# auduno/headtrackr

Measured on AMD Instinct MI355X. Metric: frames/sec full-cascade detect at 320x240, higher is better.
Workload: dtype u8; 1 GPU; C2: 256 x 320x240 RGBA frames per GPU, full BBF cascade detect (interval 5) incl. grouping + best face per frame on the host; frames_per_gpu=256, frames_total=256, width=320, height=240, batches_in_flight=3, parallelism=1 GPU

## Files before the change

### headtrackr_amd/csrc/ht_context.hip

```cpp
#include <sched.h>
#include <algorithm>
#include <cmath>
#include <cstddef>
#include <cstdlib>
#include <cstring>
#include <new>

#include "ht_internal.h"
#include "ht_hostpost.h"
#include "ht_geometry_plan.h"
#include "ht_cascade_plan.h"

static thread_local std::string g_create_err;

#include <dlfcn.h>
namespace {
struct Roctx {
    int (*push)(const char *) = nullptr;
    int (*pop)() = nullptr;
    Roctx() {
        void *h = dlopen("libroctx64.so", RTLD_NOW | RTLD_GLOBAL);
        if (!h) h = dlopen("libroctx64.so.4", RTLD_NOW | RTLD_GLOBAL);
        if (h) {
            push = reinterpret_cast<int (*)(const char *)>(dlsym(h, "roctxRangePushA"));
// ... 105 lines not shown
    ctx->timers[idx].launches++;
}

extern "C" int32_t ht_abi_version(void) { return HT_ABI_VERSION; }

extern "C" const char *ht_last_error(const ht_ctx *ctx) { return ctx ? ctx->err.c_str() : g_create_err.c_str(); }

static bool apply_options(ht_ctx *c, const std::string &opts, std::string &why) {
    size_t pos = 0;
    while (pos < opts.size()) {
        size_t end = opts.find(',', pos);
        if (end == std::string::npos) end = opts.size();
        std::string kv = opts.substr(pos, end - pos);
        pos = end + 1;
        while (!kv.empty() && (kv.front() == ' ')) kv.erase(kv.begin());
        while (!kv.empty() && (kv.back() == ' ')) kv.pop_back();
        if (kv.empty()) continue;
        const size_t eq = kv.find('=');
        const std::string key = kv.substr(0, eq), val = eq == std::string::npos ? "1" : kv.substr(eq + 1);
        char *endp = nullptr;
        const long long v = std::strtoll(val.c_str(), &endp, 10);
        if (val.empty() || (endp && *endp)) {
            why = "option '" + key + "': value is not an integer";
            return false;
        }
        const int iv = (int)std::max<long long>(std::min<long long>(v, 1ll << 30), -(1ll << 30));
        if (key == "rs_rpt") { if (iv >= 1 && iv <= HT_RS_MAX_PASSES) c->rs_rpt = iv; }
        else if (key == "rs_tailtable") c->tail_table = iv < 0 ? 0 : (iv > 2 ? 2 : (int)iv), c->tail_table_forced = true;
        else if (key == "rs_tailcap") c->rs_tailcap = (uint64_t)std::max<long long>(v, 0), c->rs_tailcap_forced = true;
        else if (key == "rs_notail") c->rs_notail = iv != 0;
        else if (key == "rs_nofast") c->rs_nofast = iv != 0;
        else if (key == "rs_nosort") c->rs_nosort = iv != 0;
        else if (key == "rs_bands") c->rs_bands = iv != 0;
        else if (key == "rs_gennames") c->rs_gennames = iv != 0;
        else if (key == "rs_minwg") c->rs_min_wgs = std::max(1, iv);
        else if (key == "rs_k") c->dbg_rs_k = iv;
        else if (key == "rs_group") { if (iv >= 1 && iv <= 64) c->rs_group = iv, c->rs_group_forced = true; }
        else if (key == "early_scan") c->early_scan = iv != 0;
        else if (key == "force_exact") c->dbg_force_exact = iv;
        else if (key == "deep_bias") c->deep_bias = (uint32_t)std::max(0, iv);
        else if (key == "deep_v") c->dbg_deep_v = iv;
        else if (key == "cs_flags") c->cs_flags = iv != 0;
        else if (key == "cs_sync_ring") c->cs_sync_ring = iv != 0;
        else if (key == "cs_pairs_force") c->cs_pairs_force = iv != 0;
        else if (key == "cs_pairs_cluster") c->cs_pairs_cluster = iv != 0;
        else if (key == "fp_sparse") c->fp_sparse = iv != 0;
        else if (key == "deep_grid") c->deep_grid = std::max(1, iv);
        else if (key == "split") c->opt_split = std::max(1, iv);
        else if (key == "cs_fused_min") c->cs_fused_min_streams = std::max(1, iv);
        else if (key == "cs_fused_nt") c->cs_fused_nt = iv;
        else if (key == "cs_keep_hist") c->cs_keep_hist = iv != 0;
        else if (key == "cs_seq_fused") c->cs_seq_fused = iv != 0;
        else if (key == "cs_cluster") c->cs_cluster = iv != 0;
        else if (key == "cs_cluster_min_px") c->cs_cluster_min_px = (uint32_t)std::max(0, iv);
        else if (key == "cs_region") c->cs_region_cap = std::min(40960, std::max(0, iv));
        else if (key == "cs_barrier_budget") c->cs_barrier_budget = std::max(1ll, v);
        else if (key == "graph_max_frames") c->graph_max_frames = std::max(0, iv);
        else if (key == "host_threads") c->host_threads = std::min(64, std::max(0, iv));
        else if (key == "force_rccl") c->force_rccl = iv != 0;
        else if (key == "group_cap") c->grp_cap_opt = std::max(1, iv);
#ifdef HT_DEBUG_KNOBS
        else if (key == "stop_stage") c->dbg_stop_stage = iv;
        else if (key == "cs_iters") c->dbg_cs_iters = std::min(10, std::max(0, iv));
        else if (key == "rs_maxgen") c->rs_maxgen = iv;
#endif
        else {
// ... 169 lines not shown
    ht_cs_best_free(c);
    ht_cs_faces_free(c);
    ht_group_free(c);
    if (c->d_gather) (void)hipFree(c->d_gather);
    for (auto &a : release) {
        if (a.orphan) {
            (void)hipSetDevice(a.device);
            (void)hipDeviceSynchronize();
        }
        (void)hipFree(a.p);
    }
    (void)hipSetDevice(c->device);
    for (auto &t : c->timers)
        for (auto &p : t.pending) (void)hipEventDestroy(p.first), (void)hipEventDestroy(p.second);
    if (c->own_stream && c->stream) (void)hipStreamDestroy(c->stream);
    delete c;
}


static ht_status set_geometry_impl(ht_ctx *c, int32_t width, int32_t height, int32_t max_batch, const int32_t *level_dims, int n, int upto) {
    c->W = width;
    c->H = height;
    c->max_batch = max_batch;
    c->nlevels = n;
    c->upto = upto;

    HtPlanInputs in;
    in.interval = c->interval, in.next = c->next, in.cw = c->cascade.cw, in.ch = c->cascade.ch;
    in.rs_rpt = c->rs_rpt, in.rs_nofast = c->rs_nofast, in.rs_nosort = c->rs_nosort, in.rs_notail = c->rs_notail;
    in.rs_tailcap = c->rs_tailcap, in.rs_tailcap_forced = c->rs_tailcap_forced;
    in.tail_table = c->tail_table, in.tail_table_forced = c->tail_table_forced;
    in.early_scan = c->early_scan, in.aux_stream = c->aux_stream != nullptr;
    in.queue_capacity_cfg = c->queue_capacity_cfg;
    HtGeometryPlan &P = c->plan;
    std::string why;
    ht_status st = ht_plan_geometry(in, width, height, max_batch, level_dims, n, upto, &P, &why);
    if (st != HT_OK) return ht_fail(c, st, why);

    c->d_gen_blocks.assign(P.gens.size(), nullptr);
    for (size_t g = 1; g < P.gens.size(); g++)
        if ((st = upload_table(c, c->d_gen_blocks[g], P.gen_tiles[g])) != HT_OK) return st;
    HT_HIP(c, hipMalloc(&c->d_levels, sizeof(HtDevLevel) * HT_MAX_LEVELS));
    HT_HIP(c, hipMemcpy(c->d_levels, P.levels, sizeof(HtDevLevel) * n, hipMemcpyHostToDevice));
    if (hipMalloc(&c->d_arena, P.arena_stride * (uint64_t)max_batch) != hipSuccess)
        return ht_fail(c, HT_ERR_NOMEM, "ht_set_geometry: hipMalloc(pyramid arena) failed");
    HT_HIP(c, hipMemset(c->d_arena, 0, P.arena_stride * (uint64_t)max_batch));
    if ((st = upload_table(c, c->d_tail_jobs, P.tail_jobs)) != HT_OK || (st = upload_table(c, c->d_tail_prefix, P.tail_prefix)) != HT_OK ||
        (st = upload_table(c, c->d_tail_taps, P.tail_taps)) != HT_OK || (st = upload_table(c, c->d_tail_taps_fast, P.tail_taps_fast)) != HT_OK ||
        (st = upload_table(c, c->d_tail_tapref, P.tail_tapref)) != HT_OK || (st = upload_table(c, c->d_tile_recs, P.tile_recs)) != HT_OK ||
        (st = upload_table(c, c->d_scales, P.scales)) != HT_OK)
        return st;
    if (hipMalloc(&c->d_queue, (size_t)P.queue_capacity * sizeof(HtQueueEntry) + HT_DEEP_CTR_BYTES) != hipSuccess)
        return ht_fail(c, HT_ERR_NOMEM, "ht_set_geometry: hipMalloc(survivor queue) failed");
    return HT_OK;
}

extern "C" ht_status ht_set_geometry(ht_ctx *c, int32_t width, int32_t height, int32_t max_batch, const int32_t *level_dims,
                                     int32_t nlevels_in) {
    if (!c) return HT_ERR_INVALID;
    if (width <= 0 || height <= 0 || width > 16384 || height > 16384 || max_batch <= 0)
        return ht_fail(c, HT_ERR_INVALID, "ht_set_geometry: width/height must be 1..16384 and max_batch > 0");
    HT_HIP(c, hipSetDevice(c->device));
    const int upto = (int)std::floor(std::log((double)std::min(c->cascade.cw, c->cascade.ch)) / std::log(ht_scale_of(c->interval)));
    const int n = upto + c->next * 2;
    if (n > HT_MAX_LEVELS) return ht_fail(c, HT_ERR_INVALID, "ht_set_geometry: too many pyramid levels");
    if (level_dims && nlevels_in != n) return ht_fail(c, HT_ERR_INVALID, "ht_set_geometry: level_dims has the wrong number of levels");
// ... 631 lines not shown
```

### headtrackr_amd/csrc/ht_geometry_plan.h

```cpp
#pragma once

#include <algorithm>
#include <cmath>
#include <cstring>
#include <string>
#include <vector>

#include "ht_hostpost.h"
#include "ht_plan_types.h"

static inline uint64_t align_up(uint64_t v, uint64_t a) { return (v + a - 1) / a * a; }

static HtTap ht_host_tap(int i, double r, int s, int origin) {
    double f = ((double)i + 0.5) * r;
    f = f + (-0.5);
    f = f < 0.0 ? 0.0 : f;
    const double fmax = (double)(s - 1);
    f = f > fmax ? fmax : f;
    const double af = std::floor(f);
    HtTap tp;
    tp.a = origin + (int)af;
    tp.b = origin + std::min((int)af + 1, s - 1);
    tp.t = f - af;
    tp.u = 1.0 - tp.t;
// ... 55 lines not shown
        j.dst_stride = D.stride;
        j.sx = sx, j.sy = sy, j.sw = sw, j.sh = sh;
        j.dw = dw, j.dh = dh;
        j.cw = D.w, j.ch = D.h;
        if (sw <= 0 || sh <= 0 || dw <= 0 || dh <= 0) {
            j.dw = j.dh = 0;
            j.sw = j.sh = 1;
            j.rx = j.ry = 1;
        } else {
            j.rx = (double)sw / (double)dw;
            j.ry = (double)sh / (double)dh;
        }
        p->gens[g].push_back(j);
    };
    for (int i = 1; i < n; i++) {
        const HtDevLevel &D = p->levels[i];
        if (i <= in.interval) {
            add_job(gen[i], 0, i, 0, 0, 0, p->levels[0].w, p->levels[0].h, D.w, D.h);
        } else {
            const HtDevLevel &S = p->levels[i - next];
            add_job(gen[i], i - next, i, 0, 0, 0, S.w, S.h, D.w, D.h);
            if (i >= 2 * next) {
                add_job(gen[i], i - next, i, 1, 1, 0, S.w - 1, S.h, D.w - 2, D.h);
                add_job(gen[i], i - next, i, 2, 0, 1, S.w, S.h - 1, D.w, D.h - 2);
                add_job(gen[i], i - next, i, 3, 1, 1, S.w - 1, S.h - 1, D.w - 2, D.h - 2);
            }
        }
    }
}

static std::vector<HtResampleJob> ht_plan_gen_tiles(const HtPlanInputs &in, const std::vector<HtResampleJob> &jobs) {
    std::vector<HtResampleJob> tiles;
    for (auto &j : jobs) {
        int npmax = 1;
        for (int t = 2; t <= std::min(in.rs_rpt, HT_RS_MAX_PASSES); t++)
            if ((int)std::ceil(16.0 * t * j.ry) + 3 <= HT_RS_SRC_ROWS) npmax = t;
        const int passes = (j.ch + 15) / 16, nby = (passes + npmax - 1) / npmax, nbx = (j.cw + 63) / 64;
        int pass0 = 0;
        for (int y = 0; y < nby; y++) {
            const int np = passes / nby + (y < passes % nby ? 1 : 0);
            for (int x = 0; x < nbx; x++) {
                HtResampleJob t = j;
                t.bx = (uint16_t)x, t.pass0 = (uint16_t)pass0, t.np = (uint16_t)np;
                t.pad = in.rs_nofast ? 2 : (uint16_t)((j.dw > 0 && j.sw == 2 * j.dw && j.sh == 2 * j.dh) ? 1 : 0);
                const int X0 = 64 * x, Y0 = 16 * pass0, ncols = std::min(64, j.dw - X0), nrows = std::min(16 * np, j.dh - Y0);
                if (ncols > 0 && nrows > 0) {
                    t.ex_xa = ht_host_tap(X0, j.rx, j.sw, j.sx).a & ~15;
                    t.ex_ya = ht_host_tap(Y0, j.ry, j.sh, j.sy).a;
                    t.ex_sw16 = (ht_host_tap(X0 + ncols - 1, j.rx, j.sw, j.sx).b - t.ex_xa) / 16 + 1;
                    t.ex_sh = ht_host_tap(Y0 + nrows - 1, j.ry, j.sh, j.sy).b - t.ex_ya + 1;
                    bool fit = t.ex_sw16 * 16 <= 160;
                    for (int w = 0; w < 4; w++) {
                        const int r0 = std::min(4 * np * w, nrows - 1), r1 = std::min(4 * np * (w + 1) - 1, nrows - 1);
                        const int bya = ht_host_tap(Y0 + r0, j.ry, j.sh, j.sy).a - t.ex_ya;
                        const int bsh = ht_host_tap(Y0 + r1, j.ry, j.sh, j.sy).b - (t.ex_ya + bya) + 1;
                        if (bya < 0 || bya > 255 || bsh < 1 || bsh > HT_RSB_ROWS) fit = false;
                        t.band_ya4 |= (uint32_t)(bya & 0xff) << (8 * w), t.band_sh4 |= (uint32_t)(bsh & 0xff) << (8 * w);
                    }
                    if (fit) t.pad |= 4;
                }
                tiles.push_back(t);
            }
            pass0 += np;
        }
    }
    if (!in.rs_nosort)
        std::stable_sort(tiles.begin(), tiles.end(), [](const HtResampleJob &a, const HtResampleJob &b) {
            if (a.src_off != b.src_off) return a.src_off < b.src_off;
            const int ya = (int)(16.0 * a.pass0 * a.ry), yb = (int)(16.0 * b.pass0 * b.ry);
            if (ya / 32 != yb / 32) return ya < yb;
            return a.bx < b.bx;
        });
    return tiles;
}

static void ht_plan_tail(const HtPlanInputs &in, int max_batch, HtGeometryPlan *p) {
    const int ngen = (int)p->gens.size();
    constexpr int HT_SMALL_BATCH = 48;
    const uint64_t tail_cap = in.rs_tailcap_forced ? in.rs_tailcap : (max_batch <= HT_SMALL_BATCH ? 4000u : in.rs_tailcap);
    p->tail_table = in.tail_table_forced ? in.tail_table : ((max_batch <= 128 && max_batch > HT_SMALL_BATCH) ? 1 : 0);
    p->tail_first_gen = 0;
    if (in.rs_notail) return;
    int g0 = ngen;
    uint64_t px = 0;
    for (int g = ngen - 1; g >= 1; g--) {
        uint64_t gp = 0;
        for (auto &j : p->gens[g]) gp += (uint64_t)j.cw * j.ch;
        if (p->gens[g].size() > (size_t)HT_TAIL_MAX_JOBS || px + gp > tail_cap) break;
        px += gp;
        g0 = g;
    }
    if (!(ngen - g0 >= 2 && ngen - g0 <= HT_TAIL_MAX_GENS)) return;
    std::vector<HtResampleJob> &tj = p->tail_jobs;
    std::vector<uint32_t> &pref = p->tail_prefix;
    HtTailGens &T = p->tail;
    std::memset(&T, 0, sizeof(T));
    T.ngen = ngen - g0;
    for (int g = g0; g < ngen; g++) {
        T.job_begin[g - g0] = (int32_t)tj.size();
        uint32_t groups = 0;
        for (auto &j : p->gens[g]) {
            tj.push_back(j);
            pref.push_back(groups);
            groups += (uint32_t)((j.cw + 3) / 4) * (uint32_t)j.ch;
// ... 128 lines not shown
```

### headtrackr_amd/csrc/ht_internal.h

```cpp
#pragma once

#include <hip/hip_runtime.h>
#include <stdint.h>

#include <atomic>
#include <string>
#include <vector>

#include "headtrackr_hip.h"

#include "ht_cascade_types.h"

#include "ht_plan_types.h"

constexpr int HT_TAIL_LDS_TAPS = 4096;

struct HtBlockRef {
    uint16_t item;
    uint16_t bx, by;
    uint16_t pad;
};

struct alignas(16) HtQueueEntry {
    uint32_t frame;
// ... 75 lines not shown
    bool builtin_cascade = false;
    uint32_t deep_bias = 1;
    int dbg_stop_stage = -1, dbg_force_exact = 0, dbg_deep_v = 4, deep_grid = 192;
    HtDevStage *d_stages = nullptr;
    int opt_split = 0;

    int W = 0, H = 0, max_batch = 0, nlevels = 0, upto = 0;
    HtGeometryPlan plan;
    HtDevLevel *d_levels = nullptr;
    uint8_t *d_arena = nullptr;
    std::vector<HtResampleJob *> d_gen_blocks;
    HtTileRec *d_tile_recs = nullptr;
    HtScanScale *d_scales = nullptr;
    HtResampleJob *d_tail_jobs = nullptr;
    uint32_t *d_tail_prefix = nullptr;
    HtTap *d_tail_taps = nullptr;
    HtTapFast *d_tail_taps_fast = nullptr;
    HtTailTapRef *d_tail_tapref = nullptr;
    bool deep_attr_set = false;
    int tail_table = 1;
    bool tail_table_forced = false;
    bool rs_nofast = false, rs_nosort = false, rs_notail = false, rs_gennames = false;
    uint64_t rs_tailcap = 32768;
    bool rs_tailcap_forced = false;
    int rs_maxgen = 1 << 30;
    bool force_rccl = false;
    int host_threads = -1;
    int rs_min_wgs = 1536;
    int dbg_rs_k = 0;
    int rs_group = 8;
    bool rs_group_forced = false;
    int rs_rpt = 4;
    bool rs_bands = true;

    uint8_t *d_frames_own = nullptr;
    size_t d_frames_own_bytes = 0;
    uint8_t *d_frames_back = nullptr;
    size_t d_frames_back_bytes = 0;
    int back_n = 0;
    hipStream_t copy_stream = nullptr;
    hipEvent_t ev_copy_done = nullptr, ev_front_free = nullptr;
    const uint8_t *d_frames = nullptr;
    size_t frame_stride = 0;
    int nframes = 0;
    std::atomic<bool> capturing{false};
    int graph_max_frames = 256;
    std::vector<HtDetectGraph> graphs;
    uint64_t graph_launches = 0;
    int64_t requeue_flags = -1;
    int enq_nframes = 0;

    uint32_t hit_capacity = 1u << 20, queue_capacity_cfg = 0;
    ht_hit *d_hits = nullptr;
    HtQueueEntry *d_queue = nullptr;
    HtCounters *d_counters = nullptr;
    uint32_t spec_hint = 0;
    HtCounters h_counters;
    uint8_t *h_pinned = nullptr;
    unsigned long long *d_stats = nullptr;
    unsigned long long h_stage_in[64] = {0};
    std::vector<ht_hit> h_collect_hits;
    std::vector<uint32_t> h_collect_counts;
    std::vector<ht_hit> h_raw_hits;
    std::vector<ht_hit> h_ordered_hits;
    std::vector<uint32_t> h_frame_start;
    bool stats_enqueued = false;
// ... 224 lines not shown
```

### headtrackr_amd/csrc/ht_plan_types.h

```cpp
#pragma once

#include <stdint.h>

#include <vector>

#include "headtrackr_hip.h"

struct HtDevLevel {
    int32_t w, h, stride;
    uint32_t off[4];
};

constexpr int HT_TAIL_MAX_GENS = 8;
constexpr int HT_TAIL_MAX_JOBS = 32;
struct HtTailGens {
    int32_t ngen;
    int32_t job_begin[HT_TAIL_MAX_GENS + 1];
    uint32_t groups[HT_TAIL_MAX_GENS];
    uint32_t tap_begin[HT_TAIL_MAX_GENS + 1];
};

struct HtTap {
    double t, u;
    int32_t a, b;
};
struct HtTapFast {
    int32_t a;
    float tf;
};
struct HtTailTapRef {
    uint32_t col, row;
    uint32_t mode;
    uint32_t pad;
};

constexpr int HT_RS_SRC_ROWS = 75;
constexpr int HT_RS_MAX_PASSES = 4;
struct HtResampleJob {
    uint32_t src_off, dst_off;
    int32_t src_stride, dst_stride;
    int32_t sx, sy, sw, sh;
    int32_t dw, dh;
    int32_t cw, ch;
    uint16_t bx, pass0;
    uint16_t np, pad;
    double rx, ry;
    int32_t ex_xa, ex_ya;
    int32_t ex_sw16, ex_sh;
    uint32_t band_ya4, band_sh4;
};
constexpr int HT_RSB_ROWS = 24;

constexpr int HT_SCAN_TXH = 64;
constexpr int HT_SCAN_TYH = 32;
struct HtScanScale {
    int32_t l0, l1, l2;
    int32_t qw, qh;
    int32_t tw2, th2;
    int32_t ntx, nty;
    uint32_t tile_begin;
    uint32_t div_magic;
    uint32_t win_begin;
};

struct alignas(64) HtTileRec {
    uint32_t off0, off1, off2[4];
    uint32_t sh0, sh1, sh2;
    uint32_t origin;
    uint32_t size;
    uint32_t tw2_l0;
    uint32_t div_magic;
    uint32_t strip_magic;
    uint32_t pad[2];
};
static_assert(sizeof(HtTileRec) == 64, "HtTileRec");

struct HtPlanInputs {
    int interval, next;
    uint32_t cw, ch;
    int rs_rpt;
    bool rs_nofast, rs_nosort, rs_notail;
    uint64_t rs_tailcap;
    bool rs_tailcap_forced;
    int tail_table;
    bool tail_table_forced;
    bool early_scan, aux_stream;
    uint32_t queue_capacity_cfg;
};

struct HtGeometryPlan {
    HtDevLevel levels[HT_MAX_LEVELS] = {};
    uint64_t arena_stride = 0;
    uint64_t pyr_bytes = 0, windows_per_frame = 0;
    std::vector<std::vector<HtResampleJob>> gens;
    std::vector<std::vector<HtResampleJob>> gen_tiles;
    std::vector<uint32_t> gen_blocks;
    int tail_first_gen = 0;
    int tail_table = 0;
    std::vector<HtResampleJob> tail_jobs;
    std::vector<uint32_t> tail_prefix;
    std::vector<HtTap> tail_taps;
    std::vector<HtTapFast> tail_taps_fast;
    std::vector<HtTailTapRef> tail_tapref;
    HtTailGens tail = {};
    std::vector<HtScanScale> scales;
    std::vector<HtTileRec> tile_recs;
    uint32_t tiles_per_frame = 0;
    int early_gen = 0;
    uint32_t early_tiles = 0;
    uint32_t queue_capacity = 0;
};
```

### headtrackr_amd/csrc/ht_pyramid.hip

```cpp
#include <cstdio>
#include <cstdlib>
#include <cstring>
#include <type_traits>

#include "ht_internal.h"
#include "ht_resample_tap.h"
#define HT_GRAY_FN __device__ __forceinline__
#include "ht_gray.h"

namespace {

__device__ __forceinline__ bool xcd_item(uint32_t per_frame, uint32_t nframes, uint32_t *frame, uint32_t *item) {
    const uint32_t chunk = gridDim.x >> 3;
    const uint32_t t = (blockIdx.x & 7u) * chunk + (blockIdx.x >> 3);
    if (t >= per_frame * nframes) return false;
    *frame = t / per_frame;
    *item = t - *frame * per_frame;
    return true;
}

__device__ __forceinline__ uint32_t gray_of(uint32_t px) { return ht_gray_of(px); }

template <bool GRAY_IN_R, bool WB>
__global__ __launch_bounds__(256) void k_gray_linear(const uint8_t *__restrict__ frames, size_t frame_stride,
// ... 71 lines not shown

typedef unsigned int rs_u32x4 __attribute__((ext_vector_type(4)));
typedef float rs_f2 __attribute__((ext_vector_type(2)));
__device__ __forceinline__ uint4 rs_buf_load16(__amdgpu_buffer_rsrc_t r, uint32_t voff, uint32_t soff) {
    const rs_u32x4 v = __builtin_amdgcn_raw_buffer_load_b128(r, voff, soff, 0);
    return make_uint4(v.x, v.y, v.z, v.w);
}

template <typename PTR>
__device__ __forceinline__ uint32_t rs_pixels4(PTR r0, PTR r1, const RsTap (&cx)[4], const RsTap &ry, int xoff, int npx) {
    uint32_t o = 0;
#pragma unroll
    for (int k = 0; k < 4; k++) {
        if (k < npx) {
            const int ia = cx[k].a - xoff, ib = cx[k].b - xoff;
            const double top = __dadd_rn(__dmul_rn((double)r0[ia], cx[k].u), __dmul_rn((double)r0[ib], cx[k].t));
            const double bot = __dadd_rn(__dmul_rn((double)r1[ia], cx[k].u), __dmul_rn((double)r1[ib], cx[k].t));
            const double vv = __dadd_rn(__dmul_rn(top, ry.u), __dmul_rn(bot, ry.t));
            const int q = (int)__builtin_rint(vv);
            o |= (uint32_t)q << (8 * k);
        }
    }
    return o;
}

#define RS_LDS_BARRIER()                                                     \
    do {                                                                     \
        __builtin_amdgcn_fence(__ATOMIC_RELEASE, "workgroup", "local");      \
        __builtin_amdgcn_s_barrier();                                        \
        __builtin_amdgcn_fence(__ATOMIC_ACQUIRE, "workgroup", "local");      \
    } while (0)
#define RS_LD1(ptr_) __hip_atomic_load((ptr_), __ATOMIC_RELAXED, __HIP_MEMORY_SCOPE_WORKGROUP)

__device__ __forceinline__ uint32_t rs_pixel_f64(const uint8_t *p, const uint8_t *p1, double cu, double ct, double ru, double rt) {
    const double top = __dadd_rn(__dmul_rn((double)p[0], cu), __dmul_rn((double)p1[0], ct));
    const double bot = __dadd_rn(__dmul_rn((double)p[RS_SP], cu), __dmul_rn((double)p1[RS_SP], ct));
    const double vv = __dadd_rn(__dmul_rn(top, ru), __dmul_rn(bot, rt));
    return (uint32_t)__double2loint(__dadd_rn(vv, 6755399441055744.0));
}

constexpr float RS_EPS = 1.0f / 8192.0f;

constexpr int RS_WPS = 6;
#if defined(HT_RS_PHASES)
__device__ unsigned long long g_rs_tl[16384][8][8];
__device__ unsigned long long g_rs_launch[1024][4];
__device__ unsigned long long g_rs_tw[4096][4][6];
#define RS_WSTAMP(i)                                                                                                                  \
    do {                                                                                                                              \
        __builtin_amdgcn_sched_barrier(0);                                                                                            \
        if (rs_iter == 2u && (threadIdx.x & 63u) == 0) g_rs_tw[rs_slot & 4095u][threadIdx.x >> 6][i] = __builtin_readcyclecounter(); \
        __builtin_amdgcn_sched_barrier(0);                                                                                            \
    } while (0)
#define HT_RS_TIMELINE 1
#define RS_SUB(i)                                                                       \
    do {                                                                                \
        __builtin_amdgcn_sched_barrier(0);                                              \
        if (threadIdx.x == 0) g_rs_tl[rs_slot][7][i] = __builtin_readcyclecounter();    \
        __builtin_amdgcn_sched_barrier(0);                                              \
    } while (0)
#define RS_STAMP(i)                                                                     \
    do {                                                                                \
        __builtin_amdgcn_sched_barrier(0);                                              \
        if (threadIdx.x == 0) g_rs_tl[rs_slot][rs_iter & 7u][i] = __builtin_readcyclecounter(); \
        __builtin_amdgcn_sched_barrier(0);                                              \
    } while (0)
#elif defined(HT_RS_TIMELINE)
__device__ unsigned long long g_rs_timeline[1 << 16][8];
#define RS_STAMP(i)                                                                     \
// ... 264 lines not shown
        int ytl = yt;
        asm volatile("" : "+v"(ytl));
#pragma unroll
        for (int q = 0; q < RPT; q++) {
            const int y = ytl + 16 * q;
            uint32_t o = 0;
            if (drawn && q < np && y < Jm.dh && npx > 0) {
                const RsTap ry = rs_tap(y, Jm.ry, Jm.sh, Jm.sy);
                o = rs_pixels4<const uint8_t *>(src + (size_t)ry.a * Jm.src_stride, src + (size_t)ry.b * Jm.src_stride, cx, ry, 0, npx);
            }
            if (q < np && y < Jm.ch && x0 < Jm.dst_stride) *reinterpret_cast<uint32_t *>(frame + Jm.dst_off + (size_t)y * Jm.dst_stride + x0) = o;
        }
    }
}

constexpr int RSB_WPS = 8;
constexpr int RSB_BAND = 4096;
#if defined(HT_RS_PHASES)
__device__ unsigned long long g_rsb_ph[256][8];
#define RSB_T(var_)                                     \
    do {                                                \
        __builtin_amdgcn_sched_barrier(0);              \
        var_ = __builtin_readcyclecounter();            \
        __builtin_amdgcn_sched_barrier(0);              \
    } while (0)
#else
#define RSB_T(var_)
#endif
typedef __attribute__((address_space(3))) void rs_lds_void;
template <int RPT>
__global__ __launch_bounds__(256, RSB_WPS) void k_resample_bands(const HtResampleJob *__restrict__ tiles, uint8_t *__restrict__ arena,
                                                                    uint64_t arena_stride, uint32_t blocks_per_frame, uint32_t ngroups,
                                                                    uint32_t nframes, uint32_t group_frames) {
    constexpr int TH = 16 * RPT;
    __shared__ __attribute__((aligned(16))) uint8_t s_src[4 * RSB_BAND];
    __shared__ RsTap s_col[RS_TW], s_row[TH];
    uint32_t gidx, blk;
    if (!xcd_item(blocks_per_frame, ngroups, &gidx, &blk)) return;
#ifdef HT_RS_PHASES
    unsigned long long rsb_t_entry = 0, rsb_t0 = 0, rsb_t1 = 0, rsb_t2 = 0, rsb_t3 = 0, rsb_t4 = 0, rsb_acc[7] = {0, 0, 0, 0, 0, 0, 0};
    RSB_T(rsb_t_entry);
#endif
    const HtResampleJob J = tiles[blk];
    const uint32_t f0 = gidx * group_frames, f1 = min(f0 + group_frames, nframes);
    const int tid = (int)threadIdx.x;
    const int np = (int)J.np;
    const int X0 = (int)J.bx * RS_TW, Y0 = (int)J.pass0 * 16;
    uint8_t *frame = arena + (uint64_t)f0 * arena_stride;
    const int ncols = min(RS_TW, J.dw - X0), nrows = min(16 * np, J.dh - Y0);
    const uint32_t mode = J.pad;
    if ((mode & 4u) && ncols > 0 && nrows > 0) {
        const int w = __builtin_amdgcn_readfirstlane(tid >> 6), l = tid & 63;
        const int xa = J.ex_xa, sw16 = J.ex_sw16;
        const int yaw = J.ex_ya + (int)((J.band_ya4 >> (8 * w)) & 0xffu);
        const int bsh = (int)((J.band_sh4 >> (8 * w)) & 0xffu);
        uint8_t *const band = s_src + w * RSB_BAND;
        uint32_t voff[4];
        bool on[4];
#pragma unroll
        for (int i = 0; i < 4; i++) {
            const int c = i * 64 + l, row = (c * 205) >> 11, col = c - row * 10;
            on[i] = col < sw16 && row < bsh;
            voff[i] = J.src_off + (uint32_t)((yaw + row) * J.src_stride + xa + 16 * col);
        }
        uint64_t fbase = reinterpret_cast<uint64_t>(frame);
#define RS_FRAME_RSRC(base_) __builtin_amdgcn_make_buffer_rsrc(reinterpret_cast<void *>(base_), 0, (int)0xffffffffu, 0x00020000)
#define RSB_DMA(fr_, soff_)                                                                                                              \
    do {                                                                                                                                 \
        _Pragma("unroll") for (int i = 0; i < 4; i++) if (on[i])                                                                         \
            __builtin_amdgcn_raw_ptr_buffer_load_lds(fr_, (rs_lds_void *)(band + i * 1024), 16, voff[i], soff_, 0, 0);                   \
    } while (0)
        {
            const __amdgpu_buffer_rsrc_t fr = RS_FRAME_RSRC(fbase);
            RSB_DMA(fr, 0u);
            if (tid < ncols) s_col[tid] = rs_tap(X0 + tid, J.rx, J.sw, J.sx);
            if (tid >= 64 && tid - 64 < nrows) s_row[tid - 64] = rs_tap(Y0 + tid - 64, J.ry, J.sh, J.sy);
        }
        __syncthreads();
        const int cbase = (l & 15) * 4, x0 = X0 + cbase;
        const int yt = Y0 + 4 * np * w + (l >> 4);
        const int npx = min(4, J.dw - x0);
        int ia[4];
        float ctf[4];
#pragma unroll
        for (int k = 0; k < 4; k++) {
            const RsTap *ct = &s_col[min(cbase + k, ncols - 1)];
            ia[k] = ct->a - xa, ctf[k] = (float)ct->t;
        }
        uint32_t one = 1u;
        asm volatile("" : "+s"(one));
        const float thr = (mode & 2u) ? -1.0f : 0.5f - RS_EPS;
        const int dh = J.dh, ch = J.ch, dst_stride = J.dst_stride;
        const uint32_t doff = J.dst_off + (uint32_t)(yt * dst_stride + x0);
        const uint32_t pxmask = npx >= 4 ? 0xffffffffu : (npx <= 0 ? 0u : ((1u << (8 * npx)) - 1u));
        const int ia8 = npx > 0 ? ia[0] : 0;
        auto frames = [&](auto NPc, auto BOXc) {
            constexpr int NP = decltype(NPc)::value;
            constexpr bool BOX = decltype(BOXc)::value;
            uint32_t roff[NP];
            float rtf[NP];
            bool st[NP], rv[NP];
#pragma unroll
            for (int q = 0; q < NP; q++) {
                const int y = yt + 4 * q;
                const RsTap *ry = &s_row[min(y - Y0, nrows - 1)];
                roff[q] = (uint32_t)((ry->a - yaw) * RS_SP + w * RSB_BAND);
                rtf[q] = (float)ry->t;
                rv[q] = y < dh;
                st[q] = y < ch && x0 < dst_stride;
            }
            for (uint32_t f = f0; f < f1; f++) {
                asm volatile("" : "+s"(fbase));
                const __amdgpu_buffer_rsrc_t fr = RS_FRAME_RSRC(fbase);
                fbase += arena_stride;
#pragma unroll
                for (int q = 0; q < NP; q++) asm volatile("" : "+v"(roff[q]));
#ifdef HT_RS_PHASES
                if (f == f0 && w == 0) rsb_acc[5] = 1ull, rsb_acc[6] = __builtin_readcyclecounter() - rsb_t_entry;
#endif
                RSB_T(rsb_t0);
                uint32_t o[NP];
                if (BOX) {
#pragma unroll
                    for (int q = 0; q < NP; q++) {
                        const uint8_t *row = s_src + roff[q] + ia8;
                        const uint2 A = *reinterpret_cast<const uint2 *>(row), B = *reinterpret_cast<const uint2 *>(row + RS_SP);
                        uint32_t oq = 0;
#pragma unroll
                        for (int k = 0; k < 4; k++) {
                            const uint32_t a = k < 2 ? A.x : A.y, b = k < 2 ? B.x : B.y;
                            const uint32_t g = __builtin_amdgcn_perm(b, a, (k & 1) ? 0x07060302u : 0x05040100u);
                            const uint32_t sum = __builtin_amdgcn_sad_u8(g, 0u, 0u);
                            oq = __builtin_amdgcn_cvt_pk_u8_f32(__builtin_rintf((float)sum * 0.25f), k, oq);
                        }
                        o[q] = rv[q] ? (oq & pxmask) : 0u;
                    }
                } else {
                    uint32_t T[16];
#pragma unroll
                    for (int q = 0; q < NP; q++) {
                        const uint8_t *row_ = s_src + roff[q];
#pragma unroll
                        for (int k = 0; k < 4; k++) {
                            const uint8_t *p_ = row_ + ia[k];
                            T[4 * k] = p_[0], T[4 * k + 1] = RS_LD1(p_ + 1), T[4 * k + 2] = p_[RS_SP], T[4 * k + 3] = RS_LD1(p_ + RS_SP + 1);
                        }
                        __builtin_amdgcn_sched_barrier(0);
                        float d[4];
                        uint32_t oq = 0;
#pragma unroll
                        for (int k = 0; k < 4; k++) {
                            const float p00 = (float)T[4 * k], p01 = (float)T[4 * k + 1], p10 = (float)T[4 * k + 2], p11 = (float)T[4 * k + 3];
                            const rs_f2 lo2 = {p00, p10}, hi2 = {p01, p11}, ct2 = {ctf[k], ctf[k]};
                            const rs_f2 tb = __builtin_elementwise_fma(ct2, hi2 - lo2, lo2);
                            const float top = tb.x, bot = tb.y;
                            const float v = __builtin_fmaf(rtf[q], bot - top, top);
                            const float r = __builtin_rintf(v);
                            d[k] = v - r;
                            oq = __builtin_amdgcn_cvt_pk_u8_f32(r, k, oq);
                        }
                        const float dmq = __builtin_fmaxf(__builtin_fmaxf(__builtin_fabsf(d[0]), __builtin_fabsf(d[1])), __builtin_fmaxf(__builtin_fabsf(d[2]), __builtin_fabsf(d[3])));
                        if (dmq >= thr) {
                            uint32_t roff_f = roff[q];
                            int yrel = yt - Y0, cb = cbase;
                            asm volatile("" : "+v"(roff_f), "+v"(yrel), "+v"(cb));
                            const RsTap *ry = &s_row[min(yrel + 4 * q, nrows - 1)];
                            const uint8_t *rowf = s_src + roff_f;
#pragma unroll
                            for (int k = 0; k < 4; k++) {
                                if (__builtin_fabsf(d[k]) >= thr) {
                                    const RsTap *ct = &s_col[min(cb + k, ncols - 1)];
                                    oq &= ~(0xffu << (8 * k));
                                    oq |= rs_pixel_f64(rowf + ia[k], rowf + ia[k] + one, ct->u, ct->t, ry->u, ry->t) << (8 * k);
                                }
                            }
                        }
                        o[q] = rv[q] ? (oq & pxmask) : 0u;
                    }
                }
#ifdef HT_RS_PHASES
#pragma unroll
                for (int q = 0; q < NP; q++) asm volatile("" ::"v"(o[q]));
#endif
                RSB_T(rsb_t1);
                if (f + 1 < f1) {
                    __builtin_amdgcn_s_waitcnt(0xc07f);
                    RSB_DMA(fr, (uint32_t)arena_stride);
                    RSB_T(rsb_t2);
                    __builtin_amdgcn_s_waitcnt(0x0f70);
                    RSB_T(rsb_t3);
                }
#pragma unroll
                for (int q = 0; q < NP; q++)
                    if (st[q]) __builtin_amdgcn_raw_buffer_store_b32(o[q], fr, doff, (uint32_t)(4 * q * dst_stride), 0);
#ifdef HT_RS_PHASES
                RSB_T(rsb_t4);
                if (f + 1 < f1) {
                    rsb_acc[0] += 1ull, rsb_acc[1] += rsb_t1 - rsb_t0, rsb_acc[2] += rsb_t2 - rsb_t1, rsb_acc[3] += rsb_t3 - rsb_t2, rsb_acc[4] += rsb_t4 - rsb_t3;
                }
#endif
            }
#ifdef HT_RS_PHASES
            if (l == 0) {
#pragma unroll
                for (int i = 0; i < 7; i++)
                    if (rsb_acc[i]) atomicAdd(&g_rsb_ph[blockIdx.x & 255u][i], rsb_acc[i]);
            }
#endif
        };
        using std::integral_constant;
        if (mode & 1u) {
            switch (np) {
                case 1: frames(integral_constant<int, 1>{}, integral_constant<bool, true>{}); break;
                case 2: frames(integral_constant<int, 2>{}, integral_constant<bool, true>{}); break;
                case 3: frames(integral_constant<int, 3>{}, integral_constant<bool, true>{}); break;
                default: frames(integral_constant<int, RPT>{}, integral_constant<bool, true>{}); break;
            }
        } else {
            switch (np) {
                case 1: frames(integral_constant<int, 1>{}, integral_constant<bool, false>{}); break;
                case 2: frames(integral_constant<int, 2>{}, integral_constant<bool, false>{}); break;
                case 3: frames(integral_constant<int, 3>{}, integral_constant<bool, false>{}); break;
                default: frames(integral_constant<int, RPT>{}, integral_constant<bool, false>{}); break;
            }
        }
#undef RSB_DMA
#undef RS_FRAME_RSRC
        return;
    }
    const HtResampleJob &Jm = tiles[blk];
    const int x0 = X0 + (tid & 15) * 4, yt = Y0 + (tid >> 4);
    const int npx = min(4, Jm.dw - x0);
    const bool drawn = ncols > 0 && nrows > 0;
    RsTap cx[4];
#pragma unroll
    for (int k = 0; k < 4; k++) cx[k] = rs_tap(min(x0 + k, X0 + max(ncols, 1) - 1), Jm.rx, Jm.sw, Jm.sx);
    for (uint32_t f = f0; f < f1; f++, frame += arena_stride) {
        const uint8_t *src = frame + Jm.src_off;
        int ytl = yt;
        asm volatile("" : "+v"(ytl));
#pragma unroll
        for (int q = 0; q < RPT; q++) {
            const int y = ytl + 16 * q;
            uint32_t o = 0;
            if (drawn && q < np && y < Jm.dh && npx > 0) {
                const RsTap ry = rs_tap(y, Jm.ry, Jm.sh, Jm.sy);
                o = rs_pixels4<const uint8_t *>(src + (size_t)ry.a * Jm.src_stride, src + (size_t)ry.b * Jm.src_stride, cx, ry, 0, npx);
            }
            if (q < np && y < Jm.ch && x0 < Jm.dst_stride) *reinterpret_cast<uint32_t *>(frame + Jm.dst_off + (size_t)y * Jm.dst_stride + x0) = o;
        }
    }
}

constexpr int TAIL_NT = 1024;
constexpr int TAIL_U = 1;
constexpr int TAIL_SMALL_WPS = 8;
template <bool LDS_TAPS, int WPS>
__global__ __launch_bounds__(TAIL_NT, WPS) void k_resample_tail(const HtResampleJob *__restrict__ jobs, const uint32_t *__restrict__ prefix,
                                                          const HtTailTapRef *__restrict__ tapref, const HtTapFast *__restrict__ tfast,
                                                          const HtTap *__restrict__ tfull, const HtTailGens G, uint8_t *__restrict__ arena,
                                                          uint64_t arena_stride, uint32_t nframes) {
    __shared__ HtResampleJob s_jobs[HT_TAIL_MAX_JOBS];
    __shared__ HtTailTapRef s_ref[HT_TAIL_MAX_JOBS];
    __shared__ uint32_t s_pref[HT_TAIL_MAX_JOBS + 1];
    __shared__ HtTapFast s_taps[LDS_TAPS ? HT_TAIL_LDS_TAPS : 1];
    uint32_t fidx, item;
    if (!xcd_item(1u, nframes, &fidx, &item)) return;
    uint8_t *frame = arena + (uint64_t)fidx * arena_stride;
    const int tid = (int)threadIdx.x;
    for (int g = 0; g < G.ngen; g++) {
        const int jb = G.job_begin[g], nj = G.job_begin[g + 1] - jb;
        const uint32_t total = G.groups[g];
        {
            const uint32_t *src32 = reinterpret_cast<const uint32_t *>(jobs + jb);
            uint32_t *dst32 = reinterpret_cast<uint32_t *>(s_jobs);
            for (int i = tid; i < nj * (int)(sizeof(HtResampleJob) / 4); i += TAIL_NT) dst32[i] = src32[i];
// ... 359 lines not shown
```

Before: 1.181 million frames/s.

## Add narrow tile shapes for resample band tiles on partial-width columns

The pyramid resample band kernel gains two narrower, taller tile shapes (32 and 16 columns wide, with matching LDS pitches and band row limits). The planner uses them for the leftover columns of a level whose width is not a multiple of 64, so those columns no longer occupy a full 64-wide tile that is partly idle. The kernel is templated on shape, and waves with no rows to process exit early. The cost is more template instantiations, a larger kernel, and more complex tap and band planning.

```diff
diff --git a/headtrackr_amd/csrc/ht_context.hip b/headtrackr_amd/csrc/ht_context.hip
--- a/headtrackr_amd/csrc/ht_context.hip
+++ b/headtrackr_amd/csrc/ht_context.hip
@@ -161,6 +161,7 @@
         else if (key == "rs_nofast") c->rs_nofast = iv != 0;
         else if (key == "rs_nosort") c->rs_nosort = iv != 0;
         else if (key == "rs_bands") c->rs_bands = iv != 0;
+        else if (key == "rs_shapes") c->rs_shapes = iv != 0;
         else if (key == "rs_gennames") c->rs_gennames = iv != 0;
         else if (key == "rs_minwg") c->rs_min_wgs = std::max(1, iv);
         else if (key == "rs_k") c->dbg_rs_k = iv;
@@ -396,6 +397,7 @@
     in.tail_table = c->tail_table, in.tail_table_forced = c->tail_table_forced;
     in.early_scan = c->early_scan, in.aux_stream = c->aux_stream != nullptr;
     in.queue_capacity_cfg = c->queue_capacity_cfg;
+    in.rs_shapes = (c->rs_bands && c->rs_shapes) ? 1 : 0;
     HtGeometryPlan &P = c->plan;
     std::string why;
     ht_status st = ht_plan_geometry(in, width, height, max_batch, level_dims, n, upto, &P, &why);
diff --git a/headtrackr_amd/csrc/ht_geometry_plan.h b/headtrackr_amd/csrc/ht_geometry_plan.h
--- a/headtrackr_amd/csrc/ht_geometry_plan.h
+++ b/headtrackr_amd/csrc/ht_geometry_plan.h
@@ -111,36 +111,58 @@
 static std::vector<HtResampleJob> ht_plan_gen_tiles(const HtPlanInputs &in, const std::vector<HtResampleJob> &jobs) {
     std::vector<HtResampleJob> tiles;
     for (auto &j : jobs) {
+        auto tile = [&](int s, int x, int pass0, int np) {
+            const int CW = 64 >> s, RW = 4 << s, X0 = x * (s ? 16 : 64);
+            HtResampleJob t = j;
+            t.bx = (uint16_t)x, t.pass0 = (uint16_t)pass0, t.np = (uint16_t)np;
+            t.pad = in.rs_nofast ? 2 : (uint16_t)((j.dw > 0 && j.sw == 2 * j.dw && j.sh == 2 * j.dh) ? 1 : 0);
+            t.pad |= (uint16_t)(s << HT_RSB_SHAPE_SHIFT);
+            const int Y0 = 16 * pass0, ncols = std::min(CW, j.dw - X0), nrows = std::min(4 * RW * np, j.dh - Y0);
+            if (ncols > 0 && nrows > 0) {
+                t.ex_xa = ht_host_tap(X0, j.rx, j.sw, j.sx).a & ~15;
+                t.ex_ya = ht_host_tap(Y0, j.ry, j.sh, j.sy).a;
+                t.ex_sw16 = (ht_host_tap(X0 + ncols - 1, j.rx, j.sw, j.sx).b - t.ex_xa) / 16 + 1;
+                t.ex_sh = ht_host_tap(Y0 + nrows - 1, j.ry, j.sh, j.sy).b - t.ex_ya + 1;
+                bool fit = t.ex_sw16 * 16 <= HT_RSB_PITCH[s];
+                for (int w = 0; w < 4; w++) {
+                    const int r0 = std::min(RW * np * w, nrows - 1), r1 = std::min(RW * np * (w + 1) - 1, nrows - 1);
+                    const int bya = ht_host_tap(Y0 + r0, j.ry, j.sh, j.sy).a - t.ex_ya;
+                    const int bsh = ht_host_tap(Y0 + r1, j.ry, j.sh, j.sy).b - (t.ex_ya + bya) + 1;
+                    if (bya < 0 || bya > 255 || bsh < 1 || bsh > HT_RSB_BAND_ROWS[s]) fit = false;
+                    t.band_ya4 |= (uint32_t)(bya & 0xff) << (8 * w), t.band_sh4 |= (uint32_t)(bsh & 0xff) << (8 * w);
+                }
+                if (fit) t.pad |= 4;
+            }
+            tiles.push_back(t);
+        };
         int npmax = 1;
         for (int t = 2; t <= std::min(in.rs_rpt, HT_RS_MAX_PASSES); t++)
             if ((int)std::ceil(16.0 * t * j.ry) + 3 <= HT_RS_SRC_ROWS) npmax = t;
-        const int passes = (j.ch + 15) / 16, nby = (passes + npmax - 1) / npmax, nbx = (j.cw + 63) / 64;
+        const int passes = (j.ch + 15) / 16, nby = (passes + npmax - 1) / npmax;
+        const int rem = in.rs_shapes ? j.cw % 64 : 0;
+        const int narrow = rem == 0 || rem > 48 ? 0 : (rem <= 16 ? 4 : (rem <= 32 ? 2 : 6));
+        const int nbx = narrow ? j.cw / 64 : (j.cw + 63) / 64;
         int pass0 = 0;
         for (int y = 0; y < nby; y++) {
             const int np = passes / nby + (y < passes % nby ? 1 : 0);
-            for (int x = 0; x < nbx; x++) {
-                HtResampleJob t = j;
-                t.bx = (uint16_t)x, t.pass0 = (uint16_t)pass0, t.np = (uint16_t)np;
-                t.pad = in.rs_nofast ? 2 : (uint16_t)((j.dw > 0 && j.sw == 2 * j.dw && j.sh == 2 * j.dh) ? 1 : 0);
-                const int X0 = 64 * x, Y0 = 16 * pass0, ncols = std::min(64, j.dw - X0), nrows = std::min(16 * np, j.dh - Y0);
-                if (ncols > 0 && nrows > 0) {
-                    t.ex_xa = ht_host_tap(X0, j.rx, j.sw, j.sx).a & ~15;
-                    t.ex_ya = ht_host_tap(Y0, j.ry, j.sh, j.sy).a;
-                    t.ex_sw16 = (ht_host_tap(X0 + ncols - 1, j.rx, j.sw, j.sx).b - t.ex_xa) / 16 + 1;
-                    t.ex_sh = ht_host_tap(Y0 + nrows - 1, j.ry, j.sh, j.sy).b - t.ex_ya + 1;
-                    bool fit = t.ex_sw16 * 16 <= 160;
-                    for (int w = 0; w < 4; w++) {
-                        const int r0 = std::min(4 * np * w, nrows - 1), r1 = std::min(4 * np * (w + 1) - 1, nrows - 1);
-                        const int bya = ht_host_tap(Y0 + r0, j.ry, j.sh, j.sy).a - t.ex_ya;
-                        const int bsh = ht_host_tap(Y0 + r1, j.ry, j.sh, j.sy).b - (t.ex_ya + bya) + 1;
-                        if (bya < 0 || bya > 255 || bsh < 1 || bsh > HT_RSB_ROWS) fit = false;
-                        t.band_ya4 |= (uint32_t)(bya & 0xff) << (8 * w), t.band_sh4 |= (uint32_t)(bsh & 0xff) << (8 * w);
-                    }
-                    if (fit) t.pad |= 4;
-                }
-                tiles.push_back(t);
-            }
+            for (int x = 0; x < nbx; x++) tile(0, x, pass0, np);
             pass0 += np;
+        }
+        int X0 = 64 * nbx;
+        for (int s = 1; s < HT_RSB_SHAPES; s++) {
+            if (!(narrow >> s & 1)) continue;
+            const int RW = 4 << s;
+            int nmax = 1;
+            for (int t = 2; t <= std::min(in.rs_rpt, HT_RSB_MAX_NP[s]); t++)
+                if ((int)std::ceil((double)(RW * t) * j.ry) + 3 <= HT_RSB_BAND_ROWS[s]) nmax = t;
+            const int sp = (j.ch + 4 * RW - 1) / (4 * RW), sby = (sp + nmax - 1) / nmax;
+            int p0 = 0;
+            for (int y = 0; y < sby; y++) {
+                const int np = sp / sby + (y < sp % sby ? 1 : 0);
+                tile(s, X0 / 16, p0, np);
+                p0 += np << s;
+            }
+            X0 += 64 >> s;
         }
     }
     if (!in.rs_nosort)
@@ -148,7 +170,7 @@
             if (a.src_off != b.src_off) return a.src_off < b.src_off;
             const int ya = (int)(16.0 * a.pass0 * a.ry), yb = (int)(16.0 * b.pass0 * b.ry);
             if (ya / 32 != yb / 32) return ya < yb;
-            return a.bx < b.bx;
+            return ht_rs_tile_x0(a) < ht_rs_tile_x0(b);
         });
     return tiles;
 }
diff --git a/headtrackr_amd/csrc/ht_internal.h b/headtrackr_amd/csrc/ht_internal.h
--- a/headtrackr_amd/csrc/ht_internal.h
+++ b/headtrackr_amd/csrc/ht_internal.h
@@ -131,6 +131,7 @@
     bool rs_group_forced = false;
     int rs_rpt = 4;
     bool rs_bands = true;
+    bool rs_shapes = true;
 
     uint8_t *d_frames_own = nullptr;
     size_t d_frames_own_bytes = 0;
diff --git a/headtrackr_amd/csrc/ht_plan_types.h b/headtrackr_amd/csrc/ht_plan_types.h
--- a/headtrackr_amd/csrc/ht_plan_types.h
+++ b/headtrackr_amd/csrc/ht_plan_types.h
@@ -50,6 +50,13 @@
     uint32_t band_ya4, band_sh4;
 };
 constexpr int HT_RSB_ROWS = 24;
+constexpr int HT_RSB_SHAPES = 3;
+constexpr int HT_RSB_SHAPE_SHIFT = 3;
+constexpr int HT_RSB_PITCH[HT_RSB_SHAPES] = {160, 96, 64};
+constexpr int HT_RSB_BAND_ROWS[HT_RSB_SHAPES] = {HT_RSB_ROWS, 41, 63};
+constexpr int HT_RSB_MAX_NP[HT_RSB_SHAPES] = {HT_RS_MAX_PASSES, 3, 1};
+static inline int ht_rs_shape(const HtResampleJob &t) { return (t.pad >> HT_RSB_SHAPE_SHIFT) & 3; }
+static inline int ht_rs_tile_x0(const HtResampleJob &t) { return (int)t.bx * (ht_rs_shape(t) ? 16 : 64); }
 
 constexpr int HT_SCAN_TXH = 64;
 constexpr int HT_SCAN_TYH = 32;
@@ -86,6 +93,7 @@
     bool tail_table_forced;
     bool early_scan, aux_stream;
     uint32_t queue_capacity_cfg;
+    int rs_shapes = 0;
 };
 
 struct HtGeometryPlan {
diff --git a/headtrackr_amd/csrc/ht_pyramid.hip b/headtrackr_amd/csrc/ht_pyramid.hip
--- a/headtrackr_amd/csrc/ht_pyramid.hip
+++ b/headtrackr_amd/csrc/ht_pyramid.hip
@@ -127,9 +127,10 @@
     } while (0)
 #define RS_LD1(ptr_) __hip_atomic_load((ptr_), __ATOMIC_RELAXED, __HIP_MEMORY_SCOPE_WORKGROUP)
 
+template <int SP = RS_SP>
 __device__ __forceinline__ uint32_t rs_pixel_f64(const uint8_t *p, const uint8_t *p1, double cu, double ct, double ru, double rt) {
     const double top = __dadd_rn(__dmul_rn((double)p[0], cu), __dmul_rn((double)p1[0], ct));
-    const double bot = __dadd_rn(__dmul_rn((double)p[RS_SP], cu), __dmul_rn((double)p1[RS_SP], ct));
+    const double bot = __dadd_rn(__dmul_rn((double)p[SP], cu), __dmul_rn((double)p1[SP], ct));
     const double vv = __dadd_rn(__dmul_rn(top, ru), __dmul_rn(bot, rt));
     return (uint32_t)__double2loint(__dadd_rn(vv, 6755399441055744.0));
 }
@@ -460,9 +461,8 @@
 __global__ __launch_bounds__(256, RSB_WPS) void k_resample_bands(const HtResampleJob *__restrict__ tiles, uint8_t *__restrict__ arena,
                                                                     uint64_t arena_stride, uint32_t blocks_per_frame, uint32_t ngroups,
                                                                     uint32_t nframes, uint32_t group_frames) {
-    constexpr int TH = 16 * RPT;
     __shared__ __attribute__((aligned(16))) uint8_t s_src[4 * RSB_BAND];
-    __shared__ RsTap s_col[RS_TW], s_row[TH];
+    __shared__ RsTap s_tap[RS_TW + 16 * RPT];
     uint32_t gidx, blk;
     if (!xcd_item(blocks_per_frame, ngroups, &gidx, &blk)) return;
 #ifdef HT_RS_PHASES
@@ -473,12 +473,18 @@
     const uint32_t f0 = gidx * group_frames, f1 = min(f0 + group_frames, nframes);
     const int tid = (int)threadIdx.x;
     const int np = (int)J.np;
-    const int X0 = (int)J.bx * RS_TW, Y0 = (int)J.pass0 * 16;
+    const uint32_t mode = J.pad;
+    const int shape = (int)((mode >> HT_RSB_SHAPE_SHIFT) & 3u);
+    const int X0 = (int)J.bx * (shape ? 16 : RS_TW), Y0 = (int)J.pass0 * 16;
     uint8_t *frame = arena + (uint64_t)f0 * arena_stride;
-    const int ncols = min(RS_TW, J.dw - X0), nrows = min(16 * np, J.dh - Y0);
-    const uint32_t mode = J.pad;
-    if ((mode & 4u) && ncols > 0 && nrows > 0) {
+    const int ncols = min(RS_TW >> shape, J.dw - X0), nrows = min((16 << shape) * np, J.dh - Y0);
+    auto bands = [&](auto SHc) {
+        constexpr int SH = decltype(SHc)::value;
+        constexpr int CG = 16 >> SH, RW = 4 << SH, SP = HT_RSB_PITCH[SH], CPR = SP / 16;
+        static_assert((HT_RSB_BAND_ROWS[SH] + 1) * SP <= RSB_BAND && 4 * CG + 4 * RW * HT_RSB_MAX_NP[SH] <= RS_TW + 16 * RPT, "shape");
+        RsTap *const s_col = s_tap, *const s_row = s_tap + 4 * CG;
         const int w = __builtin_amdgcn_readfirstlane(tid >> 6), l = tid & 63;
+        const bool idle = RW * np * w >= J.ch - Y0;
         const int xa = J.ex_xa, sw16 = J.ex_sw16;
         const int yaw = J.ex_ya + (int)((J.band_ya4 >> (8 * w)) & 0xffu);
         const int bsh = (int)((J.band_sh4 >> (8 * w)) & 0xffu);
@@ -487,16 +493,20 @@
         bool on[4];
 #pragma unroll
         for (int i = 0; i < 4; i++) {
-            const int c = i * 64 + l, row = (c * 205) >> 11, col = c - row * 10;
-            on[i] = col < sw16 && row < bsh;
+            const int c = i * 64 + l, row = c / CPR, col = c - row * CPR;
+            on[i] = col < sw16 && row < bsh && !idle;
             voff[i] = J.src_off + (uint32_t)((yaw + row) * J.src_stride + xa + 16 * col);
         }
         uint64_t fbase = reinterpret_cast<uint64_t>(frame);
 #define RS_FRAME_RSRC(base_) __builtin_amdgcn_make_buffer_rsrc(reinterpret_cast<void *>(base_), 0, (int)0xffffffffu, 0x00020000)
 #define RSB_DMA(fr_, soff_)                                                                                                              \
     do {                                                                                                                                 \
+         \
+                                                                  \
+        uint32_t band_ = (uint32_t)(uintptr_t)band;                                                                                      \
+        asm volatile("" : "+s"(band_));                                                                                                  \
         _Pragma("unroll") for (int i = 0; i < 4; i++) if (on[i])                                                                         \
-            __builtin_amdgcn_raw_ptr_buffer_load_lds(fr_, (rs_lds_void *)(band + i * 1024), 16, voff[i], soff_, 0, 0);                   \
+            __builtin_amdgcn_raw_ptr_buffer_load_lds(fr_, (rs_lds_void *)(uintptr_t)(band_ + i * 1024), 16, voff[i], soff_, 0, 0);       \
     } while (0)
         {
             const __amdgpu_buffer_rsrc_t fr = RS_FRAME_RSRC(fbase);
@@ -505,8 +515,9 @@
             if (tid >= 64 && tid - 64 < nrows) s_row[tid - 64] = rs_tap(Y0 + tid - 64, J.ry, J.sh, J.sy);
         }
         __syncthreads();
-        const int cbase = (l & 15) * 4, x0 = X0 + cbase;
-        const int yt = Y0 + 4 * np * w + (l >> 4);
+        if (idle) return;
+        const int cbase = (l & (CG - 1)) * 4, x0 = X0 + cbase;
+        const int yt = Y0 + RW * np * w + l / CG;
         const int npx = min(4, J.dw - x0);
         int ia[4];
         float ctf[4];
@@ -527,14 +538,15 @@
             constexpr bool BOX = decltype(BOXc)::value;
             uint32_t roff[NP];
             float rtf[NP];
-            bool st[NP], rv[NP];
+            bool st[NP];
+            uint32_t pxm[NP];
 #pragma unroll
             for (int q = 0; q < NP; q++) {
-                const int y = yt + 4 * q;
+                const int y = yt + RW * q;
                 const RsTap *ry = &s_row[min(y - Y0, nrows - 1)];
-                roff[q] = (uint32_t)((ry->a - yaw) * RS_SP + w * RSB_BAND);
+                roff[q] = (uint32_t)((ry->a - yaw) * SP + w * RSB_BAND);
                 rtf[q] = (float)ry->t;
-                rv[q] = y < dh;
+                pxm[q] = y < dh ? pxmask : 0u;
                 st[q] = y < ch && x0 < dst_stride;
             }
             for (uint32_t f = f0; f < f1; f++) {
@@ -552,7 +564,7 @@
 #pragma unroll
                     for (int q = 0; q < NP; q++) {
                         const uint8_t *row = s_src + roff[q] + ia8;
-                        const uint2 A = *reinterpret_cast<const uint2 *>(row), B = *reinterpret_cast<const uint2 *>(row + RS_SP);
+                        const uint2 A = *reinterpret_cast<const uint2 *>(row), B = *reinterpret_cast<const uint2 *>(row + SP);
                         uint32_t oq = 0;
 #pragma unroll
                         for (int k = 0; k < 4; k++) {
@@ -561,7 +573,7 @@
                             const uint32_t sum = __builtin_amdgcn_sad_u8(g, 0u, 0u);
                             oq = __builtin_amdgcn_cvt_pk_u8_f32(__builtin_rintf((float)sum * 0.25f), k, oq);
                         }
-                        o[q] = rv[q] ? (oq & pxmask) : 0u;
+                        o[q] = oq & pxm[q];
                     }
                 } else {
                     uint32_t T[16];
@@ -571,7 +583,7 @@
 #pragma unroll
                         for (int k = 0; k < 4; k++) {
                             const uint8_t *p_ = row_ + ia[k];
-                            T[4 * k] = p_[0], T[4 * k + 1] = RS_LD1(p_ + 1), T[4 * k + 2] = p_[RS_SP], T[4 * k + 3] = RS_LD1(p_ + RS_SP + 1);
+                            T[4 * k] = p_[0], T[4 * k + 1] = RS_LD1(p_ + 1), T[4 * k + 2] = p_[SP], T[4 * k + 3] = RS_LD1(p_ + SP + 1);
                         }
                         __builtin_amdgcn_sched_barrier(0);
                         float d[4];
@@ -592,18 +604,18 @@
                             uint32_t roff_f = roff[q];
                             int yrel = yt - Y0, cb = cbase;
                             asm volatile("" : "+v"(roff_f), "+v"(yrel), "+v"(cb));
-                            const RsTap *ry = &s_row[min(yrel + 4 * q, nrows - 1)];
+                            const RsTap *ry = &s_row[min(yrel + RW * q, nrows - 1)];
                             const uint8_t *rowf = s_src + roff_f;
 #pragma unroll
                             for (int k = 0; k < 4; k++) {
                                 if (__builtin_fabsf(d[k]) >= thr) {
                                     const RsTap *ct = &s_col[min(cb + k, ncols - 1)];
                                     oq &= ~(0xffu << (8 * k));
-                                    oq |= rs_pixel_f64(rowf + ia[k], rowf + ia[k] + one, ct->u, ct->t, ry->u, ry->t) << (8 * k);
+                                    oq |= rs_pixel_f64<SP>(rowf + ia[k], rowf + ia[k] + one, ct->u, ct->t, ry->u, ry->t) << (8 * k);
                                 }
                             }
                         }
-                        o[q] = rv[q] ? (oq & pxmask) : 0u;
+                        o[q] = oq & pxm[q];
                     }
                 }
 #ifdef HT_RS_PHASES
@@ -618,9 +630,11 @@
                     __builtin_amdgcn_s_waitcnt(0x0f70);
                     RSB_T(rsb_t3);
                 }
+                uint32_t rstep = (uint32_t)(RW * dst_stride);
+                asm volatile("" : "+s"(rstep));
 #pragma unroll
                 for (int q = 0; q < NP; q++)
-                    if (st[q]) __builtin_amdgcn_raw_buffer_store_b32(o[q], fr, doff, (uint32_t)(4 * q * dst_stride), 0);
+                    if (st[q]) __builtin_amdgcn_raw_buffer_store_b32(o[q], fr, doff, (uint32_t)q * rstep, 0);
 #ifdef HT_RS_PHASES
                 RSB_T(rsb_t4);
                 if (f + 1 < f1) {
@@ -637,27 +651,33 @@
 #endif
         };
         using std::integral_constant;
-        if (mode & 1u) {
-            switch (np) {
-                case 1: frames(integral_constant<int, 1>{}, integral_constant<bool, true>{}); break;
-                case 2: frames(integral_constant<int, 2>{}, integral_constant<bool, true>{}); break;
-                case 3: frames(integral_constant<int, 3>{}, integral_constant<bool, true>{}); break;
-                default: frames(integral_constant<int, RPT>{}, integral_constant<bool, true>{}); break;
-            }
-        } else {
-            switch (np) {
-                case 1: frames(integral_constant<int, 1>{}, integral_constant<bool, false>{}); break;
-                case 2: frames(integral_constant<int, 2>{}, integral_constant<bool, false>{}); break;
-                case 3: frames(integral_constant<int, 3>{}, integral_constant<bool, false>{}); break;
-                default: frames(integral_constant<int, RPT>{}, integral_constant<bool, false>{}); break;
-            }
-        }
+        constexpr int NPMAX = HT_RSB_MAX_NP[SH] < RPT ? HT_RSB_MAX_NP[SH] : RPT;
+        auto by_np = [&](auto BOXc) {
+            if constexpr (NPMAX >= 4) {
+                if (np >= 4) return frames(integral_constant<int, NPMAX>{}, BOXc);
+            }
+            if constexpr (NPMAX >= 3) {
+                if (np == 3) return frames(integral_constant<int, 3>{}, BOXc);
+            }
+            if constexpr (NPMAX >= 2) {
+                if (np == 2) return frames(integral_constant<int, 2>{}, BOXc);
+            }
+            return frames(integral_constant<int, 1>{}, BOXc);
+        };
+        if (mode & 1u) by_np(integral_constant<bool, true>{});
+        else by_np(integral_constant<bool, false>{});
 #undef RSB_DMA
 #undef RS_FRAME_RSRC
+    };
+    if ((mode & 4u) && ncols > 0 && nrows > 0) {
+        using std::integral_constant;
+        if (shape == 0) bands(integral_constant<int, 0>{});
+        else if (shape == 1) bands(integral_constant<int, 1>{});
+        else bands(integral_constant<int, 2>{});
         return;
     }
     const HtResampleJob &Jm = tiles[blk];
-    const int x0 = X0 + (tid & 15) * 4, yt = Y0 + (tid >> 4);
+    const int x0 = X0 + (tid & ((16 >> shape) - 1)) * 4, yt = Y0 + (tid >> (4 - shape));
     const int npx = min(4, Jm.dw - x0);
     const bool drawn = ncols > 0 && nrows > 0;
     RsTap cx[4];
@@ -669,7 +689,7 @@
         asm volatile("" : "+v"(ytl));
 #pragma unroll
         for (int q = 0; q < RPT; q++) {
-            const int y = ytl + 16 * q;
+            const int y = ytl + (16 << shape) * q;
             uint32_t o = 0;
             if (drawn && q < np && y < Jm.dh && npx > 0) {
                 const RsTap ry = rs_tap(y, Jm.ry, Jm.sh, Jm.sy);
```

After: 1.181 million frames/s. Within noise of the previous version (-0.0%).
